# robotic-vision-lab/Dual-Interactive-Implicit-Neural-Network

Hardware: AMD Instinct MI355X
Metric: decoded Mpixels/sec (DIINN implicit decoder, x4 on 256^2 LR) (higher is better)
Workload: dtype f32

## Files before the change

dual-interactive-implicit-neural-network_amd/_native.py:

```python
from __future__ import annotations

import ctypes as C
import os
import threading

PKG_DIR = os.path.dirname(os.path.abspath(__file__))
LIB_PATH = os.environ.get("DIINN_HIP_LIB") or os.path.join(PKG_DIR, "libdiinn_hip.so")

DIINN_OK = 0
ERR_INVALID_ARG, ERR_UNSUPPORTED, ERR_HIP, ERR_TOO_LARGE = 1, 2, 3, 4
SIN_ACCURATE = 0
SIN_HW = 1
SIN_HW_REDUCED = 2
SIN_DEFAULT = SIN_HW_REDUCED
ABI_VERSION = 11
PACKED_MAGIC = 0x44493038
HEAD3X3_MAGIC = 0x44494833
PACKED_MAGIC_WPU = 0x44495750
P_ALGO_DIRECT, P_ALGO_WINOGRAD, P_ALGO_DIRECT_BF16, P_ALGO_DIRECT_BF16X3 = 0, 1, 2, 3
RDN_ALGO_AUTO, RDN_ALGO_DIRECT, RDN_ALGO_WINO, RDN_ALGO_WINO4, RDN_ALGO_X3 = 0, 1, 2, 3, 4
COMPUTE_F32 = 0
COMPUTE_BF16 = 1
COMPUTE_F32_QONLY = 2
COMPUTE_BF16_FULL = 3
# ... 26 lines not shown
    "diinn_precompute_P_ex": (C.c_int, [C.c_void_p, C.c_void_p, C.c_void_p, C.c_void_p,
                                     C.c_int, C.c_int, C.c_int, C.c_int, C.c_int, C.c_int]),
    "diinn_decode_band": (C.c_int, [C.c_void_p, C.c_void_p, C.c_void_p, C.c_void_p,
                                    C.c_int, C.c_int, C.c_int, C.c_int, C.c_int, C.c_int, C.c_int, C.c_int]),
    "diinn_decode": (C.c_int, [C.c_void_p, C.c_void_p, C.c_void_p, C.c_void_p, C.c_void_p,
                               C.c_int, C.c_int, C.c_int, C.c_int, C.c_int, C.c_int, C.c_int, C.c_int]),
    "diinn_decode_band_ex": (C.c_int, [C.c_void_p, C.c_void_p, C.c_void_p, C.c_void_p,
                                       C.c_int, C.c_int, C.c_int, C.c_int, C.c_int, C.c_int, C.c_int, C.c_int, C.c_int]),
    "diinn_decode_ex": (C.c_int, [C.c_void_p, C.c_void_p, C.c_void_p, C.c_void_p, C.c_void_p,
                                  C.c_int, C.c_int, C.c_int, C.c_int, C.c_int, C.c_int, C.c_int, C.c_int, C.c_int]),
    "diinn_window_rows": (C.c_int, [C.c_int, C.c_int, C.c_int, C.c_int, C.c_int, _ip, _ip, _ip, _ip]),
    "diinn_precompute_P_win": (C.c_int, [C.c_void_p, C.c_void_p, C.c_int, C.c_int, C.c_void_p, C.c_void_p, C.c_int, C.c_int,
                                         C.c_int, C.c_int, C.c_int, C.c_int, C.c_int, C.c_int]),
    "diinn_decode_band_win": (C.c_int, [C.c_void_p, C.c_void_p, C.c_int, C.c_int, C.c_void_p, C.c_void_p, C.c_int, C.c_int,
                                        C.c_int, C.c_int, C.c_int, C.c_int, C.c_int, C.c_int, C.c_int, C.c_int, C.c_int]),
    "diinn_decode_win": (C.c_int, [C.c_void_p, C.c_void_p, C.c_int, C.c_int, C.c_void_p, C.c_void_p, C.c_int, C.c_int,
                                   C.c_void_p, C.c_int, C.c_int,
                                   C.c_int, C.c_int, C.c_int, C.c_int, C.c_int, C.c_int, C.c_int, C.c_int, C.c_int]),
    "diinn_decode_tile_win": (C.c_int, [C.c_void_p, C.c_void_p, C.c_int, C.c_int, C.c_void_p, C.c_void_p,
                                        C.c_longlong, C.c_longlong, C.c_longlong, C.c_int, C.c_int, C.c_int, C.c_int, C.c_int,
                                        C.c_int, C.c_int, C.c_int, C.c_int, C.c_int, C.c_int]),
    "diinn_cell_chain": (C.c_int, [C.c_void_p, C.c_void_p, C.c_void_p, C.c_int, C.c_int, C.c_int, C.c_int, C.c_int]),
    "diinn_head3x3_packed_floats": (C.c_size_t, []),
    "diinn_pack_head3x3": (C.c_int, [_f, _f, _f]),
    "diinn_mode4_rows": (C.c_int, [C.c_int, C.c_int, C.c_int, C.c_int, C.c_int, _ip, _ip, _ip, _ip]),
    "diinn_mode4_taps_bytes": (C.c_size_t, [C.c_int, C.c_int, C.c_int, C.c_int, C.c_int]),
    "diinn_decode_mode4_band": (C.c_int, [C.c_void_p, C.c_void_p, C.c_void_p, C.c_void_p, C.c_void_p, C.c_void_p,
                                          C.c_int, C.c_int, C.c_int, C.c_int, C.c_int, C.c_int, C.c_int, C.c_int]),
    "diinn_decode_mode4": (C.c_int, [C.c_void_p, C.c_void_p, C.c_void_p, C.c_void_p, C.c_void_p, C.c_void_p, C.c_void_p,
                                     C.c_int, C.c_int, C.c_int, C.c_int, C.c_int, C.c_int, C.c_int, C.c_int]),
    "diinn_decode_launch_info": (C.c_int, [C.c_int, C.c_int, C.c_int, C.c_int, C.c_int, _ip, _ip, _ip, _ip]),
    "diinn_p_launch_info": (C.c_int, [C.c_int, C.c_int, C.c_int, C.c_int, C.c_int, C.c_int, _ip]),
    "diinn_decode_kernel_info": (C.c_int, [C.c_int, C.c_int, C.c_int, C.c_int, C.c_int, C.c_int, C.c_int, C.c_int, _ip]),
    "diinn_debug_set": (C.c_int, [C.c_char_p, C.c_longlong]),
    "diinn_debug_get": (C.c_int, [C.c_char_p, C.POINTER(C.c_longlong)]),
    "diinn_debug_clock_probe": (C.c_int, [C.c_void_p, C.c_void_p, C.c_int, C.c_uint]),
    "diinn_metasr_packed_floats": (C.c_size_t, []),
    "diinn_metasr_pack_weights": (C.c_int, [_f, _f, _f, _f, _f]),
    "diinn_metasr_workspace_bytes": (C.c_size_t, [C.c_int, C.c_int, C.c_int]),
    "diinn_metasr_decode": (C.c_int, [C.c_void_p, C.c_void_p, C.c_void_p, C.c_void_p, C.c_void_p,
                                      C.c_int, C.c_int, C.c_int, C.c_int, C.c_int]),
    "diinn_metasr_make_axis_tables": (C.c_int, [C.c_int, C.c_int, _i32, _f, _f]),
    "diinn_conv_ksplit": (C.c_int, [C.c_void_p, C.c_void_p, C.c_longlong, C.c_int, C.c_int, C.c_void_p, C.c_void_p,
                                   C.c_void_p, C.c_longlong, C.c_void_p, C.c_longlong, C.c_void_p, C.c_longlong,
                                   C.c_int, C.c_int, C.c_int, C.c_int]),
    "diinn_rdn_packed_floats": (C.c_size_t, []),
    "diinn_rdn_planes_floats": (C.c_size_t, [C.c_int, C.c_int, C.c_int, C.c_int]),
    "diinn_rdn_forward_ex": (C.c_int, [C.c_void_p, C.c_int, C.c_void_p, C.c_void_p, C.c_void_p, C.c_void_p, C.c_void_p, C.c_void_p,
                                       C.c_void_p, C.c_void_p, C.c_void_p, C.c_int, C.c_int, C.c_int]),
    "diinn_conv_wino4_ws_status": (C.c_int, [C.c_void_p, C.c_void_p, C.c_int, _ip]),
    "diinn_sfe1_forward": (C.c_int, [C.c_void_p, C.c_void_p, C.c_int, C.c_void_p, C.c_void_p, C.c_void_p,
                                    C.c_int, C.c_int, C.c_int]),
    "diinn_conv_wino": (C.c_int, [C.c_void_p, C.c_void_p, C.c_longlong, C.c_int, C.c_void_p, C.c_void_p,
                                 C.c_void_p, C.c_longlong, C.c_void_p, C.c_longlong, C.c_int, C.c_int, C.c_int, C.c_int]),
    "diinn_conv3x3_x3": (C.c_int, [C.c_void_p, C.c_void_p, C.c_longlong, C.c_int, C.c_void_p, C.c_void_p,
                                   C.c_void_p, C.c_longlong, C.c_void_p, C.c_longlong, C.c_int, C.c_int, C.c_int, C.c_int]),
    "diinn_rdn_x3_packed_floats": (C.c_size_t, []),
    "diinn_conv_t16": (C.c_int, [C.c_void_p, C.c_void_p, C.c_longlong, C.c_int, C.c_void_p, C.c_void_p,
                                C.c_void_p, C.c_longlong, C.c_void_p, C.c_longlong, C.c_int, C.c_int, C.c_int, C.c_int]),
    "diinn_conv_t16_applies": (C.c_int, [C.c_int, C.c_int, C.c_int]),
    "diinn_conv_t16_plan": (C.c_int, [C.c_int, C.c_int, C.c_int, C.POINTER(C.c_int)]),
    "diinn_conv1x1_t16": (C.c_int, [C.c_void_p, C.c_void_p, C.c_longlong, C.c_int, C.c_void_p, C.c_void_p,
                                   C.c_void_p, C.c_longlong, C.c_void_p, C.c_longlong, C.c_void_p, C.c_longlong,
                                   C.c_int, C.c_int, C.c_int, C.c_int]),
    "diinn_rdn_wino_packed_floats": (C.c_size_t, []),
    "diinn_conv_wino4": (C.c_int, [C.c_void_p, C.c_void_p, C.c_longlong, C.c_int, C.c_void_p, C.c_void_p,
# ... 88 lines not shown
```

dual-interactive-implicit-neural-network_amd/csrc/diinn_decode.hip:

```cpp
#include "diinn_device.h"
#include <stdlib.h>

struct TagCoopF { static constexpr bool value = false; };
struct TagCoopT { static constexpr bool value = true; };

template <int SIN_MODE, bool KPART = true, bool SAVE = false, bool HEAD3 = false>
__global__ __launch_bounds__(256, 1) void decode_kernel(const DecodeParams p) {
    static_assert(!(HEAD3 && SAVE), "mode 4 is inference only");
    __shared__ __attribute__((aligned(16))) float tab[(HEAD3 ? 3 + TAPS : 6) * HID + 4];
    constexpr size_t S_WL = SAVE ? OFF_WL : OFF_WLR, S_BQ = SAVE ? OFF_BQ : OFF_BQR, S_Q0 = SAVE ? OFF_Q0 : OFF_Q0R;
    auto sine = [](float v) {
        if constexpr (SAVE) return dsin<SIN_MODE>(v); else return dsin_rev<SIN_MODE>(v);
    };
    {
        const int i = threadIdx.x & 63, part = threadIdx.x >> 6;
        const float* __restrict__ Q0s = p.Wt + S_Q0 + 4 * i;
        if (part == 0) {
            *(f32x4*)(tab + 0 * HID + 4 * i) = *(const f32x4*)(Q0s + 0 * HID);
            *(f32x4*)(tab + 1 * HID + 4 * i) = *(const f32x4*)(Q0s + 1 * HID);
        } else if (part == 1) {
            const f32x4 wr = *(const f32x4*)(Q0s + 2 * HID), bq = *(const f32x4*)(Q0s + 3 * HID);
            f32x4 t;
#pragma unroll
            for (int e = 0; e < 4; ++e) t[e] = __builtin_fmaf(wr[e], p.ratio, bq[e]);
            *(f32x4*)(tab + 2 * HID + 4 * i) = t;
        } else if constexpr (HEAD3) {
        } else if (part == 2) {
            *(f32x4*)(tab + 3 * HID + 4 * i) = *(const f32x4*)(p.Wt + OFF_L + 0 * HID + 4 * i);
            *(f32x4*)(tab + 4 * HID + 4 * i) = *(const f32x4*)(p.Wt + OFF_L + 1 * HID + 4 * i);
        } else {
            *(f32x4*)(tab + 5 * HID + 4 * i) = *(const f32x4*)(p.Wt + OFF_L + 2 * HID + 4 * i);
            if (i == 0) {
                const f32x4 bl = *(const f32x4*)(p.Wt + OFF_BL);
                const unsigned nanm = SAVE ? 0u : derived_nan_mask(p.Wt);
                *(f32x4*)(tab + 6 * HID) = or_bits(bl, nanm);
            }
        }
        if constexpr (HEAD3) {
#pragma unroll
            for (int v = threadIdx.x; v < TAPS * HID / 4; v += 256)
                *(f32x4*)(tab + 3 * HID + 4 * v) = *(const f32x4*)(p.head3 + 4 * v);
        }
    }
    const int lane = threadIdx.x & 63;
    const int wave = __builtin_amdgcn_readfirstlane(threadIdx.x >> 6);
    const int h = lane >> 5, j = lane & 31;

    int x, y, b;
    const long long ptile = (long long)blockIdx.x * 4 + wave;
    if constexpr (SAVE) {
        const long long pix = ptile * PLANE_TILE + j;
        const long long pc = pix < p.npix ? pix : p.npix - 1;
        const int hw = p.Hu * p.Wu;
        b = (int)(pc / hw);
        const int rem = (int)(pc - (long long)b * hw);
        y = rem / p.Wu;
        x = pix < p.npix ? rem - y * p.Wu : p.Wu;
    } else {
        x = p.x0 + blockIdx.x * (TILE_W * WG_TILES_X) + (wave & 1) * TILE_W + (j & (TILE_W - 1));
        y = p.y0 + blockIdx.y * (TILE_H * WG_TILES_Y) + (wave >> 1) * TILE_H + (j / TILE_W);
        b = blockIdx.z;
    }
    const bool valid = (x < p.x1) && (y < p.y1);
    __syncthreads();
    if (__builtin_amdgcn_readfirstlane((int)(__ballot(valid) == 0ull))) return;
    const int xc = x < p.Wu ? x : p.Wu - 1;
    const int yc = y < p.y1 ? y : p.y1 - 1;

    int iy, ix;
    float relh, relw;
    axis_eval(p.ah, yc, iy, relh);
    axis_eval(p.aw, xc, ix, relw);

#ifdef DIINN_STAMPS
    const size_t stamp_base = ((((size_t)blockIdx.z * gridDim.y + blockIdx.y) * gridDim.x + blockIdx.x) * 4 + wave) * 8;
    if (p.stamps && lane == 0) {
        unsigned long long rt;
        asm volatile("s_memrealtime %0\n\ts_waitcnt lgkmcnt(0)" : "=s"(rt)::"memory");
        p.stamps[stamp_base + 7] = rt;
    }
#endif
    STAMP(0);
    const float* __restrict__ Wt = p.Wt;
    const float* __restrict__ Pc = p.P + (((size_t)b * p.Prows + (iy - p.Prow0)) * p.W + ix) * PCH + 4 * h;

    const long long act_tiles = (p.npix + PLANE_TILE - 1) / PLANE_TILE;
    const unsigned act_voff = (SAVE && valid) ? 4u * j + 4u * h * PLANE_ROW_BYTES : 0xFFFFFFF0u;
    auto act_rsrc = [&](int layer) {
        return tile_rsrc(p.acts + (size_t)layer * act_tiles * ACT_ROWS * PLANE_TILE, ptile, ACT_ROWS);
    };

    float q[128];
    {
        const float* __restrict__ Q0 = tab + 4 * h;
        const __amdgpu_buffer_rsrc_t ar0 = act_rsrc(0);
#pragma unroll
        for (int m = 0; m < 8; ++m) {
#pragma unroll
            for (int g = 0; g < 4; ++g) {
                const int c0 = 32 * m + 8 * g;
                const f32x4 pv = *(const f32x4*)(Pc + c0);
                const f32x4 wh = *(const f32x4*)(Q0 + 0 * HID + c0);
                const f32x4 ww = *(const f32x4*)(Q0 + 1 * HID + c0);
                const f32x4 tq = *(const f32x4*)(Q0 + 2 * HID + c0);
#pragma unroll
                for (int e = 0; e < 4; ++e) {
                    float a = tq[e];
                    a = __builtin_fmaf(ww[e], relw, a);
                    a = __builtin_fmaf(wh[e], relh, a);
                    const float kv = relu0(pv[e]);
                    q[16 * m + 4 * g + e] = kv * sine(a);
                    if constexpr (SAVE) {
                        st_act(ar0, act_voff, (unsigned)(c0 + e) * PLANE_ROW_BYTES, kv);
                        st_act(ar0, act_voff, (unsigned)(HID + c0 + e) * PLANE_ROW_BYTES, a);
                    }
                }
            }
        }
    }

    STAMP(1);
    constexpr int PF = DECODE_PREFETCH;
    static_assert(WL_KG % PF == 0, "ring index must be static");
    const __amdgpu_buffer_rsrc_t wrs = __builtin_amdgcn_make_buffer_rsrc(
        (void*)Wt, 0, (int)(PACKED_FLOATS * sizeof(float)), 0x00020000);
    const int lane_off = lane * 16;
    int wp = (int)(S_WL * sizeof(float));
    f32x4 rk[PF], rq[PF];
#pragma unroll
    for (int d = 0; d < PF; ++d) {
        if constexpr (KPART) rk[d] = ld_piece(wrs, lane_off, wp + (2 * d + 0) * PIECE_BYTES);
        rq[d] = ld_piece(wrs, lane_off, wp + (2 * d + 1) * PIECE_BYTES);
    }
    f32x4 sk[4], sq[4];
#pragma unroll
    for (int g = 0; g < 4; ++g) {
        sk[g] = *(const f32x4*)(Pc + HID + 8 * g);
        sq[g] = *(const f32x4*)(Wt + S_BQ + 4 * h + 8 * g);
    }
#pragma unroll 1
    for (int layer = 0; layer < 3; ++layer) {
        const int nl = layer < 2 ? layer + 1 : 2;
        const float* __restrict__ Pl = Pc + (layer + 1) * HID;
        const float* __restrict__ Bq = Wt + S_BQ + layer * HID + 4 * h;
        const float* __restrict__ Pn = Pc + (nl + 1) * HID;
        const float* __restrict__ Bn = Wt + S_BQ + nl * HID + 4 * h;
        float qn[128];
        f32x16 pk, ps;
        const __amdgpu_buffer_rsrc_t arl = act_rsrc(layer + 1);
        (void)arl;
#pragma unroll
        for (int m = 0; m < 8; ++m) {
            f32x16 ak, as;
#pragma unroll
            for (int g = 0; g < 4; ++g) {
#pragma unroll
                for (int e = 0; e < 4; ++e) {
                    ak[4 * g + e] = sk[g][e];
                    as[4 * g + e] = sq[g][e];
                }
            }
#pragma unroll
            for (int kg = 0; kg < WL_KG; ++kg) {
                const int s = m * WL_KG + kg;
                const f32x4 wq = rq[s % PF];
                if constexpr (KPART) {
                    const f32x4 wk = rk[s % PF];
#pragma unroll
                    for (int e = 0; e < 4; ++e) {
                        ak = MFMA32(wk[e], q[4 * kg + e], ak);
                        as = MFMA32(wq[e], q[4 * kg + e], as);
                    }
                } else {
#pragma unroll
                    for (int e = 0; e < 4; ++e) as = MFMA32(wq[e], q[4 * kg + e], as);
                }
                if constexpr (KPART) rk[s % PF] = ld_piece(wrs, lane_off, wp + (2 * (s + PF) + 0) * PIECE_BYTES);
                rq[s % PF] = ld_piece(wrs, lane_off, wp + (2 * (s + PF) + 1) * PIECE_BYTES);
                if (kg == 4) {
#pragma unroll
                    for (int g = 0; g < 4; ++g) {
                        sk[g] = *(const f32x4*)((m < 7 ? Pl + 32 * (m + 1) : Pn) + 8 * g);
                        sq[g] = *(const f32x4*)((m < 7 ? Bq + 32 * (m + 1) : Bn) + 8 * g);
                    }
                }
                if (m > 0 && (kg & 1) == 0) {
                    const int r = kg >> 1;
                    const float kv = relu0(pk[r]);
                    qn[16 * (m - 1) + r] = kv * sine(ps[r]);
                    if constexpr (SAVE) {
                        const unsigned so = (unsigned)(32 * (m - 1) + (r & 3) + 8 * (r >> 2)) * PLANE_ROW_BYTES;
                        st_act(arl, act_voff, so, kv);
                        st_act(arl, act_voff, so + HID * PLANE_ROW_BYTES, ps[r]);
                    }
                }
            }
            pk = ak;
            ps = as;
        }
#pragma unroll
        for (int r = 0; r < 16; ++r) {
            const float kv = relu0(pk[r]);
            qn[16 * 7 + r] = kv * sine(ps[r]);
            if constexpr (SAVE) {
                const unsigned so = (unsigned)(32 * 7 + (r & 3) + 8 * (r >> 2)) * PLANE_ROW_BYTES;
                st_act(arl, act_voff, so, kv);
                st_act(arl, act_voff, so + HID * PLANE_ROW_BYTES, ps[r]);
            }
        }
#pragma unroll
        for (int i = 0; i < 128; ++i) q[i] = qn[i];
// ... 4 lines not shown
    }

    if constexpr (HEAD3) {
        float o[TAPS];
#pragma unroll
        for (int r = 0; r < TAPS; ++r) o[r] = 0.0f;
        const float* __restrict__ L = tab + 3 * HID + 4 * h;
#pragma unroll
        for (int m = 0; m < 8; ++m) {
#pragma unroll
            for (int g = 0; g < 4; ++g) {
                const int c0 = 32 * m + 8 * g;
#pragma unroll
                for (int r = 0; r < TAPS; ++r) {
                    const f32x4 l = *(const f32x4*)(L + r * HID + c0);
#pragma unroll
                    for (int e = 0; e < 4; ++e) o[r] = __builtin_fmaf(l[e], q[16 * m + 4 * g + e], o[r]);
                }
            }
        }
#pragma unroll
        for (int r = 0; r < TAPS; ++r) o[r] += __shfl_xor(o[r], 32);
        if (valid && h == 0) {
            float* t = p.out + (((long long)b * p.Orows + (y - p.Orow0)) * p.Wu + x) * TAP_STRIDE;
#pragma unroll
            for (int v = 0; v < TAP_STRIDE / 4; ++v)
                *(f32x4*)(t + 4 * v) = f32x4{o[4 * v], o[4 * v + 1], o[4 * v + 2], 4 * v + 3 < TAPS ? o[(4 * v + 3) % TAPS] : 0.0f};
        }
        STAMP(5);
        return;
    }
    float o0 = 0.0f, o1 = 0.0f, o2 = 0.0f;
    {
        const float* __restrict__ L = tab + 3 * HID + 4 * h;
#pragma unroll
        for (int m = 0; m < 8; ++m) {
#pragma unroll
            for (int g = 0; g < 4; ++g) {
                const int c0 = 32 * m + 8 * g;
                const f32x4 l0 = *(const f32x4*)(L + 0 * HID + c0);
                const f32x4 l1 = *(const f32x4*)(L + 1 * HID + c0);
                const f32x4 l2 = *(const f32x4*)(L + 2 * HID + c0);
#pragma unroll
                for (int e = 0; e < 4; ++e) {
                    const float v = q[16 * m + 4 * g + e];
                    o0 = __builtin_fmaf(l0[e], v, o0);
                    o1 = __builtin_fmaf(l1[e], v, o1);
                    o2 = __builtin_fmaf(l2[e], v, o2);
                }
            }
        }
    }
    o0 += __shfl_xor(o0, 32);
    o1 += __shfl_xor(o1, 32);
    o2 += __shfl_xor(o2, 32);
    if (valid && h == 0) {
        const long long plane = p.o_ps;
        float* o = out_px(p, b, y, x);
        o[0] = o0 + tab[6 * HID + 0];
        o[plane] = o1 + tab[6 * HID + 1];
        o[2 * plane] = o2 + tab[6 * HID + 2];
    }
    STAMP(5);
}



#define MFMA16(a, b, c) __builtin_amdgcn_mfma_f32_16x16x4f32((a), (b), (c), 0, 0, 0)
constexpr int T16_W = 4, T16_H = 4;

template <int SIN_MODE>
__global__ __launch_bounds__(256, 4) void decode_coop16_kernel(const DecodeParams p) {
    __shared__ __attribute__((aligned(16))) f32x4 qs[2][16][64];
    __shared__ __attribute__((aligned(16))) float tab[6 * HID + 4];
    {
        const int i = threadIdx.x & 63, part = threadIdx.x >> 6;
        const float* __restrict__ Q0s = p.Wt + OFF_Q0R + 4 * i;
        if (part == 0) {
            *(f32x4*)(tab + 0 * HID + 4 * i) = *(const f32x4*)(Q0s + 0 * HID);
            *(f32x4*)(tab + 1 * HID + 4 * i) = *(const f32x4*)(Q0s + 1 * HID);
        } else if (part == 1) {
            const f32x4 wr = *(const f32x4*)(Q0s + 2 * HID), bq = *(const f32x4*)(Q0s + 3 * HID);
            f32x4 t;
#pragma unroll
            for (int e = 0; e < 4; ++e) t[e] = __builtin_fmaf(wr[e], p.ratio, bq[e]);
            *(f32x4*)(tab + 2 * HID + 4 * i) = t;
        } else if (part == 2) {
            *(f32x4*)(tab + 3 * HID + 4 * i) = *(const f32x4*)(p.Wt + OFF_L + 0 * HID + 4 * i);
            *(f32x4*)(tab + 4 * HID + 4 * i) = *(const f32x4*)(p.Wt + OFF_L + 1 * HID + 4 * i);
        } else {
            *(f32x4*)(tab + 5 * HID + 4 * i) = *(const f32x4*)(p.Wt + OFF_L + 2 * HID + 4 * i);
            if (i == 0) *(f32x4*)(tab + 6 * HID) = or_bits(*(const f32x4*)(p.Wt + OFF_BL), derived_nan_mask(p.Wt));
        }
    }
    const int lane = threadIdx.x & 63;
    const int wave = __builtin_amdgcn_readfirstlane(threadIdx.x >> 6);
// ... 204 lines not shown
                    kn[16 * m + 4 * g + e] = v[e];
                }
                if (valid) *(f32x4*)(Pl + 32 * m + 8 * g) = v;
            }
        }
#pragma unroll
        for (int i = 0; i < 128; ++i) k[i] = kn[i];
        wp += (int)(WL_LAYER * sizeof(float));
    }
}


static int cell_chain_impl(void* stream, float* P_dev, const float* packed_dev, int B, int H, int W, int r0, int r1,
                           RowWin pw) {
    if (!P_dev || !packed_dev) return DIINN_ERR_INVALID_ARG;
    int st = check_dims(B, H, W);
    if (st) return st;
    if (r0 < 0 || r1 > H || r0 >= r1) return DIINN_ERR_INVALID_ARG;
    st = check_window(pw.row0, pw.rows, H, r0, r1);
    if (st) return st;
    ChainParams p{P_dev, packed_dev, B, H, W, r0, r1, pw.row0, pw.rows};
    const dim3 grid((W + TILE_W * WG_TILES_X - 1) / (TILE_W * WG_TILES_X),
                    (r1 - r0 + TILE_H * WG_TILES_Y - 1) / (TILE_H * WG_TILES_Y), B);
    if (grid.y > 65535) return DIINN_ERR_TOO_LARGE;
    hipLaunchKernelGGL(cell_chain_kernel, grid, dim3(256), 0, (hipStream_t)stream, p);
    return hip_status(hipGetLastError());
}

struct OutView { int row0, rows, col0; long long bs, ps, rs; };
static inline OutView contig(RowWin ow, int Wu) {
    return OutView{ow.row0, ow.rows, 0, 3LL * ow.rows * Wu, (long long)ow.rows * Wu, (long long)Wu};
}

struct F32Choice { int kernel; dim3 grid; };
static F32Choice f32_kernel_choice(int B, int y0, int y1, int x0, int x1) {
    const int gx = (x1 - x0 + TILE_W * WG_TILES_X - 1) / (TILE_W * WG_TILES_X);
    const int gy = (y1 - y0 + TILE_H * WG_TILES_Y - 1) / (TILE_H * WG_TILES_Y);
    const int force = (int)knob(diinn_knobs().f32_kernel);
    const int ncu = device_cus();
    const dim3 grid16((x1 - x0 + T16_W - 1) / T16_W, (y1 - y0 + T16_H - 1) / T16_H, B);
    const double t16 = (double)grid16.x * grid16.y * grid16.z, rounds = (double)(((long long)gx * gy * B + ncu - 1) / ncu);
    const bool cheaper16 = 0.0896 * t16 * (256.0 / ncu) + 25.0 < 181.1 * rounds + 3.0;
    if (grid16.y <= 65535 && (force ? force == 3 : cheaper16)) return F32Choice{DIINN_DECODE_KERNEL_LATENCY16, grid16};
    return F32Choice{DIINN_DECODE_KERNEL_THROUGHPUT, dim3(gx, gy, B)};
}

static int decode_tile_impl(void* stream, const float* P_dev, const float* packed_dev,
                            float* out_dev, int B, int H, int W, int Hu, int Wu,
                            int y0, int y1, int x0, int x1, int sin_mode, int compute, RowWin pw, OutView ov) {
    if (!compute_ok(compute))
        return DIINN_ERR_UNSUPPORTED;
    if (!P_dev || !packed_dev || !out_dev) return DIINN_ERR_INVALID_ARG;
    int st = check_dims(B, H, W);
    if (st) return st;
    if (Hu <= 0 || Wu <= 0 || y0 < 0 || y1 > Hu || y0 >= y1 || x0 < 0 || x1 > Wu || x0 >= x1) return DIINN_ERR_INVALID_ARG;
    if ((double)Hu * Wu >= 2.0e9) return DIINN_ERR_TOO_LARGE;
    {
        int r0, r1;
        st = diinn_lr_rows_for_band(H, Hu, Wu, y0, y1, &r0, &r1);
        if (st) return st;
        st = check_window(pw.row0, pw.rows, H, r0, r1);
        if (st) return st;
        st = check_window(ov.row0, ov.rows, Hu, y0, y1);
        if (st) return st;
    }
    if (ov.col0 < 0 || ov.col0 > x0 || ov.rs < (long long)(x1 - ov.col0) || ov.ps < ov.rs * (y1 - ov.row0 - 1) + (x1 - ov.col0) ||
        ov.bs < 2 * ov.ps + ov.rs * (y1 - ov.row0 - 1) + (x1 - ov.col0) || ov.bs > (1LL << 40))
        return DIINN_ERR_INVALID_ARG;
    if (sin_mode < DIINN_SIN_ACCURATE || sin_mode > DIINN_SIN_HW_REDUCED) return DIINN_ERR_UNSUPPORTED;
    const int gx = (x1 - x0 + TILE_W * WG_TILES_X - 1) / (TILE_W * WG_TILES_X);
    const int gy = (y1 - y0 + TILE_H * WG_TILES_Y - 1) / (TILE_H * WG_TILES_Y);
    const int gz = B, blk = 256;
    if (gy > 65535 || gz > 65535) return DIINN_ERR_TOO_LARGE;
    DecodeParams p;
    p.P = P_dev; p.Wt = packed_dev; p.out = out_dev;
    p.B = B; p.H = H; p.W = W; p.Hu = Hu; p.Wu = Wu; p.y0 = y0; p.y1 = y1;
    p.ratio = (float)(((double)H * (double)W) / ((double)Hu * (double)Wu));
// ... 1 lines not shown
    p.x0 = x0; p.x1 = x1; p.Ocol0 = ov.col0; p.o_bs = ov.bs; p.o_ps = ov.ps; p.o_rs = ov.rs;
    p.acts = nullptr; p.npix = 0; p.seed_cols = 0; p.xcd_runs = 0;
    for (int i = 0; i < 6; ++i) p.pg[i] = 0;
#ifdef DIINN_STAMPS
    p.stamps = g_stamps;
#endif
    const int small = diinn_uses_small_output_kernel(Hu, Wu);
    p.ah = make_axis(H, Hu, small);
    p.aw = make_axis(W, Wu, small);
    const dim3 grid(gx, gy, gz);
    if (compute == DIINN_COMPUTE_BF16 || compute == DIINN_COMPUTE_BF16_FULL)
        return launch_decode_bf16(stream, p, gx, gy, gz, sin_mode);
    if (compute == DIINN_COMPUTE_BF16X3)
        return launch_decode_bf16x3(stream, p, gx, gy, gz, sin_mode);
    if (compute == DIINN_COMPUTE_F32_QONLY) {
        if (sin_mode == DIINN_SIN_HW)
            hipLaunchKernelGGL((decode_kernel<DIINN_SIN_HW, false>), grid, dim3(blk), 0, (hipStream_t)stream, p);
        else if (sin_mode == DIINN_SIN_HW_REDUCED)
            hipLaunchKernelGGL((decode_kernel<DIINN_SIN_HW_REDUCED, false>), grid, dim3(blk), 0, (hipStream_t)stream, p);
        else
            hipLaunchKernelGGL((decode_kernel<DIINN_SIN_ACCURATE, false>), grid, dim3(blk), 0, (hipStream_t)stream, p);
        return hip_status(hipGetLastError());
    }
    const F32Choice ch = f32_kernel_choice(B, y0, y1, x0, x1);
    if (ch.kernel == DIINN_DECODE_KERNEL_LATENCY16) {
        if (sin_mode == DIINN_SIN_HW)
            hipLaunchKernelGGL(decode_coop16_kernel<DIINN_SIN_HW>, ch.grid, dim3(256), 0, (hipStream_t)stream, p);
        else if (sin_mode == DIINN_SIN_HW_REDUCED)
            hipLaunchKernelGGL(decode_coop16_kernel<DIINN_SIN_HW_REDUCED>, ch.grid, dim3(256), 0, (hipStream_t)stream, p);
        else
            hipLaunchKernelGGL(decode_coop16_kernel<DIINN_SIN_ACCURATE>, ch.grid, dim3(256), 0, (hipStream_t)stream, p);
        return hip_status(hipGetLastError());
    }
    if (sin_mode == DIINN_SIN_HW)
        hipLaunchKernelGGL(decode_kernel<DIINN_SIN_HW>, grid, dim3(blk), 0, (hipStream_t)stream, p);
    else if (sin_mode == DIINN_SIN_HW_REDUCED)
        hipLaunchKernelGGL(decode_kernel<DIINN_SIN_HW_REDUCED>, grid, dim3(blk), 0, (hipStream_t)stream, p);
    else
        hipLaunchKernelGGL(decode_kernel<DIINN_SIN_ACCURATE>, grid, dim3(blk), 0, (hipStream_t)stream, p);
    return hip_status(hipGetLastError());
}

static int decode_band_impl(void* stream, const float* P_dev, const float* packed_dev,
                            float* out_dev, int B, int H, int W, int Hu, int Wu,
                            int y0, int y1, int sin_mode, int compute, RowWin pw, RowWin ow) {
    if (Wu <= 0) return DIINN_ERR_INVALID_ARG;
    return decode_tile_impl(stream, P_dev, packed_dev, out_dev, B, H, W, Hu, Wu, y0, y1, 0, Wu, sin_mode, compute, pw,
                            contig(ow, Wu));
}

static int decode_impl(void* stream, const float* feat_dev, const float* packed_dev,
                       float* workspace_dev, float* out_dev,
                       int B, int H, int W, int Hu, int Wu, int y0, int y1, int sin_mode, int compute,
                       RowWin fw, RowWin pw, RowWin ow) {
    if (!workspace_dev) return DIINN_ERR_INVALID_ARG;

    int r0, r1;
    int st = diinn_lr_rows_for_band(H, Hu, Wu, y0, y1, &r0, &r1);
    if (st) return st;
    if (!compute_ok(compute))
        return DIINN_ERR_UNSUPPORTED;
    st = launch_P(stream, feat_dev, packed_dev, workspace_dev, B, H, W, r0, r1, 16, p_arith(compute),
                  &fw, &pw, true);
    if (st) return st;
    if (compute == DIINN_COMPUTE_F32_QONLY) {
        st = cell_chain_impl(stream, workspace_dev, packed_dev, B, H, W, r0, r1, pw);
// ... 115 lines not shown
    return decode_mode4_band_impl(stream, workspace_dev, packed_dev, head_dev, taps_dev, out_dev, B, H, W, Hu, Wu, y0, y1,
                                  sin_mode, full, RowWin{0, Hu});
}

int diinn_cell_chain(void* stream, float* P_dev, const float* packed_dev, int B, int H, int W, int r0, int r1) {
    return cell_chain_impl(stream, P_dev, packed_dev, B, H, W, r0, r1, RowWin{0, H});
}

int diinn_decode_launch_info(int B, int Hu, int Wu, int y0, int y1,
                             int* grid_x, int* grid_y, int* grid_z, int* block) {
    if (B <= 0 || Hu <= 0 || Wu <= 0 || y0 < 0 || y1 > Hu || y0 >= y1) return DIINN_ERR_INVALID_ARG;
    if (grid_x) *grid_x = (Wu + TILE_W * WG_TILES_X - 1) / (TILE_W * WG_TILES_X);
    if (grid_y) *grid_y = (y1 - y0 + TILE_H * WG_TILES_Y - 1) / (TILE_H * WG_TILES_Y);
    if (grid_z) *grid_z = B;
    if (block) *block = 256;
    return DIINN_OK;
}

int diinn_decode_kernel_info(int B, int Hu, int Wu, int y0, int y1, int x0, int x1, int compute, int info[4]) {
    if (!info || B <= 0 || Hu <= 0 || Wu <= 0 || y0 < 0 || y1 > Hu || y0 >= y1 || x0 < 0 || x1 > Wu || x0 >= x1) return DIINN_ERR_INVALID_ARG;
    if (!compute_ok(compute)) return DIINN_ERR_UNSUPPORTED;
    if (compute == DIINN_COMPUTE_F32) {
        const F32Choice ch = f32_kernel_choice(B, y0, y1, x0, x1);
        info[0] = ch.kernel; info[1] = (int)ch.grid.x; info[2] = (int)ch.grid.y; info[3] = (int)ch.grid.z;
        return DIINN_OK;
    }
    info[0] = compute == DIINN_COMPUTE_F32_QONLY ? DIINN_DECODE_KERNEL_THROUGHPUT : DIINN_DECODE_KERNEL_OTHER;
    info[1] = (x1 - x0 + TILE_W * WG_TILES_X - 1) / (TILE_W * WG_TILES_X);
    info[2] = (y1 - y0 + TILE_H * WG_TILES_Y - 1) / (TILE_H * WG_TILES_Y);
    info[3] = B;
    return DIINN_OK;
}

int diinn_decode_band(void* stream, const float* P_dev, const float* packed_dev,
                      float* out_dev, int B, int H, int W, int Hu, int Wu,
                      int y0, int y1, int sin_mode) {
    return diinn_decode_band_ex(stream, P_dev, packed_dev, out_dev, B, H, W, Hu, Wu, y0, y1, sin_mode,
                                DIINN_COMPUTE_F32);
}

int diinn_decode_band_ex(void* stream, const float* P_dev, const float* packed_dev,
                         float* out_dev, int B, int H, int W, int Hu, int Wu,
                         int y0, int y1, int sin_mode, int compute) {
    return decode_band_impl(stream, P_dev, packed_dev, out_dev, B, H, W, Hu, Wu, y0, y1, sin_mode, compute,
                            RowWin{0, H}, RowWin{0, Hu});
}

int diinn_decode_band_win(void* stream, const float* P_win_dev, int p_row0, int p_rows, const float* packed_dev,
                          float* out_win_dev, int out_row0, int out_rows,
                          int B, int H, int W, int Hu, int Wu, int y0, int y1, int sin_mode, int compute) {
    return decode_band_impl(stream, P_win_dev, packed_dev, out_win_dev, B, H, W, Hu, Wu, y0, y1, sin_mode, compute,
                            RowWin{p_row0, p_rows}, RowWin{out_row0, out_rows});
}

int diinn_decode_tile_win(void* stream, const float* P_win_dev, int p_row0, int p_rows, const float* packed_dev,
                          float* out_tile_dev, long long out_row_stride, long long out_plane_stride,
                          long long out_batch_stride, int B, int H, int W, int Hu, int Wu,
                          int y0, int y1, int x0, int x1, int sin_mode, int compute) {
    return decode_tile_impl(stream, P_win_dev, packed_dev, out_tile_dev, B, H, W, Hu, Wu, y0, y1, x0, x1, sin_mode, compute,
                            RowWin{p_row0, p_rows},
                            OutView{y0, y1 > y0 ? y1 - y0 : 1, x0, out_batch_stride, out_plane_stride, out_row_stride});
}

static int train_fwd_impl(void* stream, const float* P_dev, const float* packed_dev, float* out_dev,
                          float* acts_dev, int B, int H, int W, int Hu, int Wu, int sin_mode, bool kpart) {
    if (!P_dev || !packed_dev || !out_dev || !acts_dev) return DIINN_ERR_INVALID_ARG;
// ... 75 lines not shown
```

dual-interactive-implicit-neural-network_amd/csrc/diinn_device.h:

```cpp
#pragma once
#include <hip/hip_runtime.h>
#include <stdint.h>

#include "../../include/diinn_hip.h"
#include "diinn_layout.h"
#include "diinn_knobs.h"

using namespace diinn;

typedef float f32x4 __attribute__((ext_vector_type(4)));
typedef float f32x16 __attribute__((ext_vector_type(16)));
typedef float f32x2 __attribute__((ext_vector_type(2)));
typedef unsigned u32x2 __attribute__((ext_vector_type(2)));
template <int N> struct IC { static constexpr int value = N; };

#define MFMA32(a, b, c) __builtin_amdgcn_mfma_f32_32x32x2f32((a), (b), (c), 0, 0, 0)

template <int MODE>
__device__ __forceinline__ float dsin(float x);

template <>
__device__ __forceinline__ float dsin<DIINN_SIN_ACCURATE>(float x) {
    const float k = __builtin_rintf(x * 0.31830988618379067154f);
    float r = __builtin_fmaf(k, -3.14159274101257324219f, x);
// ... 56 lines not shown
    long long npix;
#ifdef DIINN_STAMPS
    unsigned long long* stamps;
#endif
};

#ifdef DIINN_STAMPS
#define STAMP(i)                                                                              \
    do {                                                                                      \
        __builtin_amdgcn_sched_barrier(0);                                                    \
        unsigned long long t_;                                                                \
        asm volatile("s_memtime %0\n\ts_waitcnt lgkmcnt(0)" : "=s"(t_)::"memory");           \
        __builtin_amdgcn_sched_barrier(0);                                                    \
        if (p.stamps && lane == 0) p.stamps[stamp_base + (i)] = t_;                           \
    } while (0)
#else
#define STAMP(i) do {} while (0)
#endif

__device__ __forceinline__ float* out_px(const DecodeParams& p, int b, int y, int x) {
    return p.out + (long long)b * p.o_bs + (long long)(y - p.Orow0) * p.o_rs + (x - p.Ocol0);
}

constexpr int TILE_W = 8, TILE_H = 4;
#ifndef WSTREAM_AUX
#define WSTREAM_AUX 0
#endif
#ifndef P_PREFETCH
#define P_PREFETCH 4
#endif
#ifndef DECODE_PREFETCH
#define DECODE_PREFETCH 4
#endif

__device__ __forceinline__ unsigned derived_nan_mask(const float* __restrict__ Wt) {
    return __builtin_bit_cast(unsigned, Wt[OFF_BL + 3]) == DIINN_PACKED_MAGIC ? 0u : 0x7fc00000u;
}
__device__ __forceinline__ float or_bits(float v, unsigned m) {
    return __builtin_bit_cast(float, __builtin_bit_cast(unsigned, v) | m);
}
__device__ __forceinline__ f32x4 or_bits(f32x4 v, unsigned m) {
    return f32x4{or_bits(v[0], m), or_bits(v[1], m), or_bits(v[2], m), or_bits(v[3], m)};
}

__device__ __forceinline__ float relu0(float x) { return __builtin_elementwise_maximum(x, 0.0f); }

typedef unsigned u32x4 __attribute__((ext_vector_type(4)));
__device__ __forceinline__ f32x4 ld_piece(__amdgpu_buffer_rsrc_t rsrc, int lane_off, int byte_off) {
    return __builtin_bit_cast(f32x4, __builtin_amdgcn_raw_buffer_load_b128(rsrc, lane_off, byte_off, WSTREAM_AUX));
}
constexpr int PIECE_BYTES = (int)(WL_PIECE * sizeof(float));
__device__ __forceinline__ void l2_touch(__amdgpu_buffer_rsrc_t rsrc, unsigned voff, float* sink_wave) {
    __builtin_amdgcn_raw_ptr_buffer_load_lds(rsrc, (__attribute__((address_space(3))) void*)sink_wave, 4, (int)voff, 0, 0, 0);
}
constexpr int WG_TILES_X = 2, WG_TILES_Y = 2;

constexpr int PLANE_TILE = 32;
constexpr int ACT_ROWS = 2 * HID;
constexpr unsigned PLANE_ROW_BYTES = PLANE_TILE * sizeof(float);
#ifndef ST_ACT_AUX
#define ST_ACT_AUX 2
#endif
__device__ __forceinline__ void st_act(__amdgpu_buffer_rsrc_t rsrc, unsigned voff, unsigned soff, float v) {
    __builtin_amdgcn_raw_buffer_store_b32(__builtin_bit_cast(unsigned, v), rsrc, (int)voff, (int)soff, ST_ACT_AUX);
}
struct BlockXYZ { int x, y, z; };
// ... 90 lines not shown
```

include/diinn_hip.h:

```cpp
#ifndef DIINN_HIP_H
#define DIINN_HIP_H

#include <stddef.h>
#include <stdint.h>

#ifdef __cplusplus
extern "C" {
#endif

#define DIINN_ABI_VERSION 11

#define DIINN_OK                 0
#define DIINN_ERR_INVALID_ARG    1
#define DIINN_ERR_UNSUPPORTED    2
#define DIINN_ERR_HIP            3
#define DIINN_ERR_TOO_LARGE      4

#define DIINN_IN_CHANNELS 64
#define DIINN_HIDDEN      256
#define DIINN_LAYERS      4
#define DIINN_OUT         3
#define DIINN_P_CHANNELS  (DIINN_LAYERS * DIINN_HIDDEN)

#define DIINN_SIN_ACCURATE 0
// ... 159 lines not shown
                           float* out_dev, long long out_batch_stride, int relu, int B, int H, int W,
                           float* ws_dev, size_t ws_floats);
int    diinn_conv_wino4_plan(int Cin, int B, int H, int W, int with_workspace, int info[4]);
int    diinn_conv_wino4_ws_status(void* stream, float* ws_dev, int clear, int* status);
#define DIINN_WINO4_MAX_SPLIT_WGS 256
#define DIINN_WINO4_COUNTER_BYTES 2048
size_t diinn_rdn_wino4_packed_floats(void);
int    diinn_rdn_wino4_applies(int B, int H, int W);

int    diinn_conv3x3_x3(void* stream, const float* in_dev, long long in_batch_stride, int Cin,
                        const float* packed_x3_dev, const float* bias_dev,
                        const float* res_dev, long long res_batch_stride,
                        float* out_dev, long long out_batch_stride, int relu, int B, int H, int W);
size_t diinn_rdn_x3_packed_floats(void);

int    diinn_conv_t16(void* stream, const float* in_dev, long long in_batch_stride, int Cin,
                      const float* packed_w_dev, const float* bias_dev,
                      const float* res_dev, long long res_batch_stride,
                      float* out_dev, long long out_batch_stride, int relu, int B, int H, int W);
int    diinn_conv_t16_applies(int B, int H, int W);
int    diinn_conv_t16_plan(int B, int H, int W, int info[4]);
int    diinn_conv1x1_t16(void* stream, const float* in_dev, long long in_batch_stride, int Cin,
                         const float* packed_w_dev, const float* bias_dev,
                         const float* res_dev, long long res_batch_stride,
                         float* out0_dev, long long out0_batch_stride, float* out1_dev, long long out1_batch_stride,
                         int relu, int B, int H, int W);

int diinn_decode_launch_info(int B, int Hu, int Wu, int y0, int y1,
                             int* grid_x, int* grid_y, int* grid_z, int* block);
#define DIINN_DECODE_KERNEL_THROUGHPUT 1
#define DIINN_DECODE_KERNEL_LATENCY16  3
#define DIINN_DECODE_KERNEL_OTHER      0
int diinn_decode_kernel_info(int B, int Hu, int Wu, int y0, int y1, int x0, int x1, int compute, int info[4]);
#define DIINN_P_ALGO_DIRECT      0
#define DIINN_P_ALGO_WINOGRAD    1
#define DIINN_P_ALGO_DIRECT_BF16 2
#define DIINN_P_ALGO_DIRECT_BF16X3 3
int diinn_p_launch_info(int B, int H, int W, int r0, int r1, int compute, int* algorithm);

int diinn_debug_set(const char* name, long long value);
int diinn_debug_get(const char* name, long long* value);
int diinn_debug_clock_probe(void* stream, unsigned long long* samples_dev, int n, unsigned realtime_ticks);

#ifdef __cplusplus
}
#endif
#endif
```

Baseline: 173.1.

## Add opt-in persistent resident decode kernel and MFMA layer-0 path

New measurement: 173.7 (median of 6 runs). No clear change (+0.3%).

```diff
diff --git a/dual-interactive-implicit-neural-network_amd/_native.py b/dual-interactive-implicit-neural-network_amd/_native.py
--- a/dual-interactive-implicit-neural-network_amd/_native.py
+++ b/dual-interactive-implicit-neural-network_amd/_native.py
@@ -82,6 +82,7 @@
     "diinn_decode_launch_info": (C.c_int, [C.c_int, C.c_int, C.c_int, C.c_int, C.c_int, _ip, _ip, _ip, _ip]),
     "diinn_p_launch_info": (C.c_int, [C.c_int, C.c_int, C.c_int, C.c_int, C.c_int, C.c_int, _ip]),
     "diinn_decode_kernel_info": (C.c_int, [C.c_int, C.c_int, C.c_int, C.c_int, C.c_int, C.c_int, C.c_int, C.c_int, _ip]),
+    "diinn_decode_resident_info": (C.c_int, [C.c_int, C.c_int, C.c_int, C.c_int, C.c_int, C.c_int, C.c_int, _ip]),
     "diinn_debug_set": (C.c_int, [C.c_char_p, C.c_longlong]),
     "diinn_debug_get": (C.c_int, [C.c_char_p, C.POINTER(C.c_longlong)]),
     "diinn_debug_clock_probe": (C.c_int, [C.c_void_p, C.c_void_p, C.c_int, C.c_uint]),
diff --git a/dual-interactive-implicit-neural-network_amd/csrc/diinn_decode.hip b/dual-interactive-implicit-neural-network_amd/csrc/diinn_decode.hip
--- a/dual-interactive-implicit-neural-network_amd/csrc/diinn_decode.hip
+++ b/dual-interactive-implicit-neural-network_amd/csrc/diinn_decode.hip
@@ -4,9 +4,14 @@
 struct TagCoopF { static constexpr bool value = false; };
 struct TagCoopT { static constexpr bool value = true; };
 
-template <int SIN_MODE, bool KPART = true, bool SAVE = false, bool HEAD3 = false>
+constexpr int DECODE_RESIDENT = 4;
+template <int SIN_FORM, bool KPART = true, bool SAVE = false, bool HEAD3 = false>
 __global__ __launch_bounds__(256, 1) void decode_kernel(const DecodeParams p) {
+    constexpr int SIN_MODE = SIN_FORM & 3;
+    constexpr bool RESIDENT = (SIN_FORM & DECODE_RESIDENT) != 0;
+    static_assert(SIN_FORM >= 0 && SIN_FORM < 8, "sine mode 0..2, + DECODE_RESIDENT");
     static_assert(!(HEAD3 && SAVE), "mode 4 is inference only");
+    static_assert(!RESIDENT || (KPART && !SAVE && !HEAD3), "the resident form is mode 3 inference only");
     __shared__ __attribute__((aligned(16))) float tab[(HEAD3 ? 3 + TAPS : 6) * HID + 4];
     constexpr size_t S_WL = SAVE ? OFF_WL : OFF_WLR, S_BQ = SAVE ? OFF_BQ : OFF_BQR, S_Q0 = SAVE ? OFF_Q0 : OFF_Q0R;
     auto sine = [](float v) {
@@ -56,21 +61,47 @@
         const int rem = (int)(pc - (long long)b * hw);
         y = rem / p.Wu;
         x = pix < p.npix ? rem - y * p.Wu : p.Wu;
-    } else {
+    } else if constexpr (!RESIDENT) {
         x = p.x0 + blockIdx.x * (TILE_W * WG_TILES_X) + (wave & 1) * TILE_W + (j & (TILE_W - 1));
         y = p.y0 + blockIdx.y * (TILE_H * WG_TILES_Y) + (wave >> 1) * TILE_H + (j / TILE_W);
         b = blockIdx.z;
     }
-    const bool valid = (x < p.x1) && (y < p.y1);
+    const int tile_gx = RESIDENT ? p.pg[0] : 1, tile_gy = RESIDENT ? p.pg[1] : 1;
+    const int tile_n = RESIDENT ? tile_gx * tile_gy * p.pg[2] : 1, tile_step = RESIDENT ? (int)gridDim.x : 1;
+    auto next_tile = [&](int t) {
+        while (t < tile_n) {
+            const int bx = t % tile_gx, by = (t / tile_gx) % tile_gy;
+            if (p.x0 + bx * (TILE_W * WG_TILES_X) + (wave & 1) * TILE_W < p.x1 &&
+                p.y0 + by * (TILE_H * WG_TILES_Y) + (wave >> 1) * TILE_H < p.y1) break;
+            t += tile_step;
+        }
+        return t;
+    };
+    auto tile_pixel = [&](int t, int& tx, int& ty, int& tb) {
+        const int bx = t % tile_gx, by = (t / tile_gx) % tile_gy;
+        tx = p.x0 + bx * (TILE_W * WG_TILES_X) + (wave & 1) * TILE_W + (j & (TILE_W - 1));
+        ty = p.y0 + by * (TILE_H * WG_TILES_Y) + (wave >> 1) * TILE_H + (j / TILE_W);
+        tb = t / (tile_gx * tile_gy);
+    };
+    auto cell_of = [&](int px, int py, int pb, float& rh, float& rw) -> const float* {
+        const int pxc = px < p.Wu ? px : p.Wu - 1;
+        const int pyc = py < p.y1 ? py : p.y1 - 1;
+        int ciy, cix;
+        axis_eval(p.ah, pyc, ciy, rh);
+        axis_eval(p.aw, pxc, cix, rw);
+        return p.P + (((size_t)pb * p.Prows + (ciy - p.Prow0)) * p.W + cix) * PCH + 4 * h;
+    };
+    int tile = 0;
     __syncthreads();
-    if (__builtin_amdgcn_readfirstlane((int)(__ballot(valid) == 0ull))) return;
-    const int xc = x < p.Wu ? x : p.Wu - 1;
-    const int yc = y < p.y1 ? y : p.y1 - 1;
-
-    int iy, ix;
+    if constexpr (RESIDENT) {
+        tile = next_tile((int)blockIdx.x);
+        if (tile >= tile_n) return;
+        tile_pixel(tile, x, y, b);
+    }
+    bool valid = (x < p.x1) && (y < p.y1);
+    if constexpr (!RESIDENT)
+        if (__builtin_amdgcn_readfirstlane((int)(__ballot(valid) == 0ull))) return;
     float relh, relw;
-    axis_eval(p.ah, yc, iy, relh);
-    axis_eval(p.aw, xc, ix, relw);
 
 #ifdef DIINN_STAMPS
     const size_t stamp_base = ((((size_t)blockIdx.z * gridDim.y + blockIdx.y) * gridDim.x + blockIdx.x) * 4 + wave) * 8;
@@ -82,7 +113,7 @@
 #endif
     STAMP(0);
     const float* __restrict__ Wt = p.Wt;
-    const float* __restrict__ Pc = p.P + (((size_t)b * p.Prows + (iy - p.Prow0)) * p.W + ix) * PCH + 4 * h;
+    const float* Pc = cell_of(x, y, b, relh, relw);
 
     const long long act_tiles = (p.npix + PLANE_TILE - 1) / PLANE_TILE;
     const unsigned act_voff = (SAVE && valid) ? 4u * j + 4u * h * PLANE_ROW_BYTES : 0xFFFFFFF0u;
@@ -90,9 +121,67 @@
         return tile_rsrc(p.acts + (size_t)layer * act_tiles * ACT_ROWS * PLANE_TILE, ptile, ACT_ROWS);
     };
 
+    constexpr int PF = DECODE_PREFETCH;
+    static_assert(WL_KG % PF == 0, "ring index must be static");
+    const __amdgpu_buffer_rsrc_t wrs = __builtin_amdgcn_make_buffer_rsrc(
+        (void*)Wt, 0, (int)(PACKED_FLOATS * sizeof(float)), 0x00020000);
+    const int lane_off = lane * 16;
+    constexpr int WP0 = (int)(S_WL * sizeof(float)), LAYER_BYTES = (int)(WL_LAYER * sizeof(float));
+    static_assert(LAYER_BYTES == 8 * WL_KG * 2 * PIECE_BYTES, "a layer is 8 x WL_KG steps of two pieces");
+    f32x4 rk[PF], rq[PF];
+    f32x4 sk[4], sq[4];
+    auto ring_start = [&]() {
+#pragma unroll
+        for (int d = 0; d < PF; ++d) {
+            if constexpr (KPART) rk[d] = ld_piece(wrs, lane_off, WP0 + (2 * d + 0) * PIECE_BYTES);
+            rq[d] = ld_piece(wrs, lane_off, WP0 + (2 * d + 1) * PIECE_BYTES);
+        }
+#pragma unroll
+        for (int g = 0; g < 4; ++g) {
+            sk[g] = *(const f32x4*)(Pc + HID + 8 * g);
+            sq[g] = *(const f32x4*)(Wt + S_BQ + 4 * h + 8 * g);
+        }
+    };
+    if constexpr (RESIDENT) ring_start();
+
+#pragma unroll 1
+    for (;;) {
+    int tile_nx = tile, xn = x, yn = y, bn = b;
+    float relhn = relh, relwn = relw;
+    const float* Pcn = Pc;
+    if constexpr (RESIDENT) {
+        tile_nx = next_tile(tile + tile_step);
+        if (tile_nx < tile_n) {
+            tile_pixel(tile_nx, xn, yn, bn);
+            Pcn = cell_of(xn, yn, bn, relhn, relwn);
+        }
+    }
+    int ht = h;
+    if constexpr (RESIDENT) asm volatile("" : "+v"(ht));
     float q[128];
-    {
-        const float* __restrict__ Q0 = tab + 4 * h;
+    if constexpr (!SAVE && DECODE_L0_MFMA) {
+        const float* __restrict__ Q0 = tab + 4 * ht;
+        const float* __restrict__ Qa = tab + (1 - ht) * HID + j;
+        const float rel = h ? relh : relw;
+#pragma unroll
+        for (int m = 0; m < 8; ++m) {
+            f32x16 a;
+#pragma unroll
+            for (int g = 0; g < 4; ++g) {
+                const f32x4 tq = *(const f32x4*)(Q0 + 2 * HID + 32 * m + 8 * g);
+#pragma unroll
+                for (int e = 0; e < 4; ++e) a[4 * g + e] = tq[e];
+            }
+            a = MFMA32(Qa[32 * m], rel, a);
+#pragma unroll
+            for (int g = 0; g < 4; ++g) {
+                const f32x4 pv = *(const f32x4*)(Pc + 32 * m + 8 * g);
+#pragma unroll
+                for (int e = 0; e < 4; ++e) q[16 * m + 4 * g + e] = relu0(pv[e]) * sine(a[4 * g + e]);
+            }
+        }
+    } else {
+        const float* __restrict__ Q0 = tab + 4 * ht;
         const __amdgpu_buffer_rsrc_t ar0 = act_rsrc(0);
 #pragma unroll
         for (int m = 0; m < 8; ++m) {
@@ -120,31 +209,17 @@
     }
 
     STAMP(1);
-    constexpr int PF = DECODE_PREFETCH;
-    static_assert(WL_KG % PF == 0, "ring index must be static");
-    const __amdgpu_buffer_rsrc_t wrs = __builtin_amdgcn_make_buffer_rsrc(
-        (void*)Wt, 0, (int)(PACKED_FLOATS * sizeof(float)), 0x00020000);
-    const int lane_off = lane * 16;
-    int wp = (int)(S_WL * sizeof(float));
-    f32x4 rk[PF], rq[PF];
-#pragma unroll
-    for (int d = 0; d < PF; ++d) {
-        if constexpr (KPART) rk[d] = ld_piece(wrs, lane_off, wp + (2 * d + 0) * PIECE_BYTES);
-        rq[d] = ld_piece(wrs, lane_off, wp + (2 * d + 1) * PIECE_BYTES);
-    }
-    f32x4 sk[4], sq[4];
-#pragma unroll
-    for (int g = 0; g < 4; ++g) {
-        sk[g] = *(const f32x4*)(Pc + HID + 8 * g);
-        sq[g] = *(const f32x4*)(Wt + S_BQ + 4 * h + 8 * g);
-    }
+    int wp = WP0;
+    if constexpr (!RESIDENT) ring_start();
 #pragma unroll 1
     for (int layer = 0; layer < 3; ++layer) {
         const int nl = layer < 2 ? layer + 1 : 2;
+        const bool wrap = RESIDENT && layer == 2;
+        const int wpx = wrap ? WP0 - LAYER_BYTES : wp;
         const float* __restrict__ Pl = Pc + (layer + 1) * HID;
         const float* __restrict__ Bq = Wt + S_BQ + layer * HID + 4 * h;
-        const float* __restrict__ Pn = Pc + (nl + 1) * HID;
-        const float* __restrict__ Bn = Wt + S_BQ + nl * HID + 4 * h;
+        const float* __restrict__ Pn = wrap ? Pcn + HID : Pc + (nl + 1) * HID;
+        const float* __restrict__ Bn = Wt + S_BQ + (wrap ? 0 : nl) * HID + 4 * h;
         float qn[128];
         f32x16 pk, ps;
         const __amdgpu_buffer_rsrc_t arl = act_rsrc(layer + 1);
@@ -175,8 +250,9 @@
 #pragma unroll
                     for (int e = 0; e < 4; ++e) as = MFMA32(wq[e], q[4 * kg + e], as);
                 }
-                if constexpr (KPART) rk[s % PF] = ld_piece(wrs, lane_off, wp + (2 * (s + PF) + 0) * PIECE_BYTES);
-                rq[s % PF] = ld_piece(wrs, lane_off, wp + (2 * (s + PF) + 1) * PIECE_BYTES);
+                const int wr = RESIDENT && s + PF >= 8 * WL_KG ? wpx : wp;
+                if constexpr (KPART) rk[s % PF] = ld_piece(wrs, lane_off, wr + (2 * (s + PF) + 0) * PIECE_BYTES);
+                rq[s % PF] = ld_piece(wrs, lane_off, wr + (2 * (s + PF) + 1) * PIECE_BYTES);
                 if (kg == 4) {
 #pragma unroll
                     for (int g = 0; g < 4; ++g) {
@@ -247,7 +323,7 @@
     }
     float o0 = 0.0f, o1 = 0.0f, o2 = 0.0f;
     {
-        const float* __restrict__ L = tab + 3 * HID + 4 * h;
+        const float* __restrict__ L = tab + 3 * HID + 4 * ht;
 #pragma unroll
         for (int m = 0; m < 8; ++m) {
 #pragma unroll
@@ -277,6 +353,14 @@
         o[2 * plane] = o2 + tab[6 * HID + 2];
     }
     STAMP(5);
+    if constexpr (!RESIDENT) {
+        break;
+    } else {
+        if (tile_nx >= tile_n) break;
+        tile = tile_nx; x = xn; y = yn; b = bn; relh = relhn; relw = relwn; Pc = Pcn;
+        valid = (x < p.x1) && (y < p.y1);
+    }
+    }
 }
 
 
@@ -547,17 +631,24 @@
     return OutView{ow.row0, ow.rows, 0, 3LL * ow.rows * Wu, (long long)ow.rows * Wu, (long long)Wu};
 }
 
-struct F32Choice { int kernel; dim3 grid; };
+constexpr bool DECODE_RESIDENT_DEFAULT = false;
+constexpr double DECODE_RESIDENT_ROUND_US = 194.7;
+struct F32Choice { int kernel; dim3 grid; int resident; };
 static F32Choice f32_kernel_choice(int B, int y0, int y1, int x0, int x1) {
     const int gx = (x1 - x0 + TILE_W * WG_TILES_X - 1) / (TILE_W * WG_TILES_X);
     const int gy = (y1 - y0 + TILE_H * WG_TILES_Y - 1) / (TILE_H * WG_TILES_Y);
-    const int force = (int)knob(diinn_knobs().f32_kernel);
+    const int knob_v = (int)knob(diinn_knobs().f32_kernel);
+    const int force = knob_v == 4 ? 0 : knob_v;
     const int ncu = device_cus();
+    const long long tiles = (long long)gx * gy * B;
+    const bool res_ok = tiles < (1LL << 30);
+    const bool res_auto = (DECODE_RESIDENT_DEFAULT || knob_v == 4) && res_ok && tiles >= 2LL * ncu;
     const dim3 grid16((x1 - x0 + T16_W - 1) / T16_W, (y1 - y0 + T16_H - 1) / T16_H, B);
-    const double t16 = (double)grid16.x * grid16.y * grid16.z, rounds = (double)(((long long)gx * gy * B + ncu - 1) / ncu);
-    const bool cheaper16 = 0.0896 * t16 * (256.0 / ncu) + 25.0 < 181.1 * rounds + 3.0;
-    if (grid16.y <= 65535 && (force ? force == 3 : cheaper16)) return F32Choice{DIINN_DECODE_KERNEL_LATENCY16, grid16};
-    return F32Choice{DIINN_DECODE_KERNEL_THROUGHPUT, dim3(gx, gy, B)};
+    const double t16 = (double)grid16.x * grid16.y * grid16.z, rounds = (double)((tiles + ncu - 1) / ncu);
+    const bool cheaper16 = 0.0896 * t16 * (256.0 / ncu) + 25.0 < (DECODE_RESIDENT_DEFAULT && res_auto ? DECODE_RESIDENT_ROUND_US : 181.1) * rounds + 3.0;
+    if (grid16.y <= 65535 && (force ? force == 3 : cheaper16)) return F32Choice{DIINN_DECODE_KERNEL_LATENCY16, grid16, 0};
+    const bool resident = force == 2 ? res_ok : force == 0 && res_auto;
+    return F32Choice{DIINN_DECODE_KERNEL_THROUGHPUT, dim3(gx, gy, B), resident ? (int)(tiles < ncu ? tiles : ncu) : 0};
 }
 
 static int decode_tile_impl(void* stream, const float* P_dev, const float* packed_dev,
@@ -625,6 +716,17 @@
             hipLaunchKernelGGL(decode_coop16_kernel<DIINN_SIN_ACCURATE>, ch.grid, dim3(256), 0, (hipStream_t)stream, p);
         return hip_status(hipGetLastError());
     }
+    if (ch.resident) {
+        p.pg[0] = gx; p.pg[1] = gy; p.pg[2] = gz;
+        const dim3 rgrid(ch.resident);
+        if (sin_mode == DIINN_SIN_HW)
+            hipLaunchKernelGGL((decode_kernel<DIINN_SIN_HW | DECODE_RESIDENT>), rgrid, dim3(blk), 0, (hipStream_t)stream, p);
+        else if (sin_mode == DIINN_SIN_HW_REDUCED)
+            hipLaunchKernelGGL((decode_kernel<DIINN_SIN_HW_REDUCED | DECODE_RESIDENT>), rgrid, dim3(blk), 0, (hipStream_t)stream, p);
+        else
+            hipLaunchKernelGGL((decode_kernel<DIINN_SIN_ACCURATE | DECODE_RESIDENT>), rgrid, dim3(blk), 0, (hipStream_t)stream, p);
+        return hip_status(hipGetLastError());
+    }
     if (sin_mode == DIINN_SIN_HW)
         hipLaunchKernelGGL(decode_kernel<DIINN_SIN_HW>, grid, dim3(blk), 0, (hipStream_t)stream, p);
     else if (sin_mode == DIINN_SIN_HW_REDUCED)
@@ -806,6 +908,12 @@
     return DIINN_OK;
 }
 
+int diinn_decode_resident_info(int B, int Hu, int Wu, int y0, int y1, int x0, int x1, int* workgroups) {
+    if (!workgroups || B <= 0 || Hu <= 0 || Wu <= 0 || y0 < 0 || y1 > Hu || y0 >= y1 || x0 < 0 || x1 > Wu || x0 >= x1) return DIINN_ERR_INVALID_ARG;
+    *workgroups = f32_kernel_choice(B, y0, y1, x0, x1).resident;
+    return DIINN_OK;
+}
+
 int diinn_decode_band(void* stream, const float* P_dev, const float* packed_dev,
                       float* out_dev, int B, int H, int W, int Hu, int Wu,
                       int y0, int y1, int sin_mode) {
diff --git a/dual-interactive-implicit-neural-network_amd/csrc/diinn_device.h b/dual-interactive-implicit-neural-network_amd/csrc/diinn_device.h
--- a/dual-interactive-implicit-neural-network_amd/csrc/diinn_device.h
+++ b/dual-interactive-implicit-neural-network_amd/csrc/diinn_device.h
@@ -112,6 +112,9 @@
 #ifndef DECODE_PREFETCH
 #define DECODE_PREFETCH 4
 #endif
+#ifndef DECODE_L0_MFMA
+#define DECODE_L0_MFMA 1
+#endif
 
 __device__ __forceinline__ unsigned derived_nan_mask(const float* __restrict__ Wt) {
     return __builtin_bit_cast(unsigned, Wt[OFF_BL + 3]) == DIINN_PACKED_MAGIC ? 0u : 0x7fc00000u;
diff --git a/include/diinn_hip.h b/include/diinn_hip.h
--- a/include/diinn_hip.h
+++ b/include/diinn_hip.h
@@ -215,6 +215,7 @@
 #define DIINN_DECODE_KERNEL_LATENCY16  3
 #define DIINN_DECODE_KERNEL_OTHER      0
 int diinn_decode_kernel_info(int B, int Hu, int Wu, int y0, int y1, int x0, int x1, int compute, int info[4]);
+int diinn_decode_resident_info(int B, int Hu, int Wu, int y0, int y1, int x0, int x1, int* workgroups);
 #define DIINN_P_ALGO_DIRECT      0
 #define DIINN_P_ALGO_WINOGRAD    1
 #define DIINN_P_ALGO_DIRECT_BF16 2
```
